# AgoraIO-Community/Solo

Hardware: AMD Instinct MI355X
Metric: 40 ms frames/sec (encode+decode) per GPU; concurrent real-time WB streams @1/2/4/8 MI355X (higher is better)
Workload: dtype int32 fixed point (int16 PCM, Q-format arithmetic, bit-exact); 1 GPU; BASELINE configs[2]: 4096 synthetic 16 kHz WB streams, full encode -> two-description bitstream -...; streams_per_gpu=4096, input_workers=16, launch=single process

## Files before the change

solo_amd/csrc/solo_enc_nsq_row.h:

```cpp
#pragma once
#include <stddef.h>
#include "solo_enc_state.h"

#define SX_JOINT_LAMBDA 90000
#define SX_DD_MASK (SX_DD_DELAY - 1)

#if SX_NLANES == 1
#define RW_NL 12
#define RW_NS 12
#define RW_FORK(l) for (int l = 0; l < 12; l++)
#define RW_LI(l) (l)
#define RW_SI(l) (l)
#define RW_ONCE(l) 1
#define RW_IS_C(l) 1
#define RW_IS_S(l) 1
#else
#define RW_NL 1
#define RW_NS 1
#define RW_FORK(l) for (int l = SX_LANE, once_ = 1; once_; once_ = 0)
#define RW_LI(l) 0
#define RW_SI(l) 0
#define RW_ONCE(l) 1
#define RW_IS_C(l) 1
#define RW_IS_S(l) 1
#endif
#define RW_T(l) ((l) >> 2)
#define RW_K(l) ((l) & 3)
#define RW_TT(l) (RW_T(l) > 2 ? 0 : RW_T(l))
#define RW_LIVE(l) (RW_T(l) < 3)
#define RW_UNI(arr) ((arr)[0])

#if SX_NLANES == 1
#define RWK_GATHER(dst, src, idx) { i32 o_[12]; for (int q_ = 0; q_ < 12; q_++) o_[q_] = (src)[q_]; for (int q_ = 0; q_ < 12; q_++) (dst)[q_] = o_[(q_ & ~3) | (idx)[q_]]; }
#define RWK_ARG_(val, mv, mi, CMP) { for (int b_ = 0; b_ < 12; b_ += 4) { i32 bv_ = (val)[b_]; int bi_ = 0;                         \
        for (int q_ = 1; q_ < 4; q_++) if ((val)[b_ + q_] CMP bv_) { bv_ = (val)[b_ + q_]; bi_ = q_; }                                \
        for (int q_ = 0; q_ < 4; q_++) { (mv)[b_ + q_] = bv_; (mi)[b_ + q_] = bi_; } } }
#define RWK_ARGMIN(val, mv, mi) RWK_ARG_(val, mv, mi, <)
#define RWK_ARGMAX(val, mv, mi) RWK_ARG_(val, mv, mi, >)
#define RWK_SUM(val, out) { for (int b_ = 0; b_ < 12; b_ += 4) { const i32 s_ = sx_add(sx_add((val)[b_], (val)[b_ + 1]), sx_add((val)[b_ + 2], (val)[b_ + 3])); \
        for (int q_ = 0; q_ < 4; q_++) (out)[b_ + q_] = s_; } }
#define RWK_PERM(LV, idx) { i32 o_[12]; for (int q_ = 0; q_ < 12; q_++) o_[q_] = LV(q_); for (int q_ = 0; q_ < 12; q_++) LV(q_) = o_[(q_ & ~3) | (idx)[q_]]; }
#define RWK_PICK(dst, src, idx) RWK_GATHER(dst, src, idx)
#define RWS_PICK(dst, src, idx) RWK_GATHER(dst, src, idx)
#define RWS_ARGMIN(val, mv, mi) RWK_ARGMIN(val, mv, mi)
#define RWS_ARGMAX(val, mv, mi) RWK_ARGMAX(val, mv, mi)
#define RWS_SUM(val, out) RWK_SUM(val, out)
#define RWS_PERM(LV, idx) RWK_PERM(LV, idx)
#define RWT_FROM(dst, src, T) { i32 o_[4]; for (int q_ = 0; q_ < 4; q_++) o_[q_] = (src)[4 * (T) + q_]; for (int q_ = 0; q_ < 12; q_++) (dst)[q_] = o_[q_ & 3]; }
#define RWT_TO0(dst, src, T) { for (int q_ = 0; q_ < 4; q_++) (dst)[q_] = (src)[4 * (T) + q_]; }
#define RWT_SUM(dst, src) { i32 o_[4]; for (int q_ = 0; q_ < 4; q_++) o_[q_] = sx_add(sx_add((src)[q_], (src)[4 + q_]), (src)[8 + q_]); for (int q_ = 0; q_ < 12; q_++) (dst)[q_] = o_[q_ & 3]; }
#define RWT_OR(dst, src) { i32 o_[4]; for (int q_ = 0; q_ < 4; q_++) o_[q_] = (src)[q_] | (src)[4 + q_] | (src)[8 + q_]; for (int q_ = 0; q_ < 12; q_++) (dst)[q_] = o_[q_ & 3]; }
#else
#define RW_DPP(v, ctrl) __builtin_amdgcn_update_dpp(0, (v), (ctrl), 0xf, 0xf, true)
#define RW_SHR(n) (0x110 + (n))
#define RW_SHL(n) (0x100 + (n))
#define RW_ROR(n) (0x120 + (n))
SX_HD i32 rwk_sel(i32 v, i32 idx) {
    const i32 b0 = RW_DPP(v, 0x00), b1 = RW_DPP(v, 0x55), b2 = RW_DPP(v, 0xAA), b3 = RW_DPP(v, 0xFF);
    const bool o_ = (idx & 1) != 0, h_ = (idx & 2) != 0;
    const i32 lo_ = o_ ? b1 : b0, hi_ = o_ ? b3 : b2;
    return h_ ? hi_ : lo_;
}
SX_HD i32 rwk_from(i32 v, i32 src) { return __builtin_amdgcn_ds_bpermute((int)((((threadIdx.x & ~3u) | (u32)src)) << 2), v); }
SX_HD i32 rwk_first_(bool eq) {
    const unsigned long long b_ = __builtin_amdgcn_ballot_w64(eq);
    return (i32)__builtin_ctz((u32)(b_ >> (threadIdx.x & 60u)) & 15u);
}
SX_HD i32 rwk_min_(i32 v) { v = sx_min(v, RW_DPP(v, 0xB1)); return sx_min(v, RW_DPP(v, 0x4E)); }
SX_HD i32 rwk_max_(i32 v) { v = sx_max(v, RW_DPP(v, 0xB1)); return sx_max(v, RW_DPP(v, 0x4E)); }
SX_HD i32 rwk_or_(i32 v) { v |= RW_DPP(v, 0xB1); return v | RW_DPP(v, 0x4E); }
SX_HD i32 rwk_sum_(i32 v) { v = sx_add(v, RW_DPP(v, 0xB1)); return sx_add(v, RW_DPP(v, 0x4E)); }
SX_HD i32 rwk_pick_(i32 v, i32 idx) { return rwk_or_((i32)(threadIdx.x & 3u) == idx ? v : 0); }
#define RWS_ARGMIN(val, mv, mi) { const i32 m_ = rwk_min_((val)[0]); (mv)[0] = m_; (mi)[0] = rwk_first_((val)[0] == m_); }
#define RWS_ARGMAX(val, mv, mi) { const i32 m_ = rwk_max_((val)[0]); (mv)[0] = m_; (mi)[0] = rwk_first_((val)[0] == m_); }
#define RWS_PICK(dst, src, idx) { (dst)[0] = rwk_pick_((src)[0], (idx)[0]); }
#define RWS_SUM(val, out) { (out)[0] = rwk_sum_((val)[0]); }
#define RWS_PERM(LV, idx) { LV(0) = rwk_from(LV(0), (idx)[0]); }
#if defined(__HIP_DEVICE_COMPILE__) && !defined(RW_CENTRE_SERIAL)
#define RW_ROW_C 1
#endif
#define RWK_GATHER(dst, src, idx) { (dst)[0] = rwk_sel((src)[0], (idx)[0]); }
#define RWK_PICK(dst, src, idx) RWS_PICK(dst, src, idx)
#define RWK_PERM(LV, idx) RWS_PERM(LV, idx)
#define RWK_ARGMIN(val, mv, mi) RWS_ARGMIN(val, mv, mi)
#define RWK_ARGMAX(val, mv, mi) RWS_ARGMAX(val, mv, mi)
SX_HD i32 rwt_from0(i32 v) { const u32 t_ = threadIdx.x & 12u; const i32 a_ = RW_DPP(v, RW_SHR(4)), b_ = RW_DPP(v, RW_SHR(8)); return t_ == 4u ? a_ : (t_ == 8u ? b_ : v); }
SX_HD i32 rwt_from1(i32 v) { const u32 t_ = threadIdx.x & 12u; const i32 a_ = RW_DPP(v, RW_SHL(4)), b_ = RW_DPP(v, RW_SHR(4)); return t_ == 0u ? a_ : (t_ == 8u ? b_ : v); }
SX_HD i32 rwt_from2(i32 v) { const u32 t_ = threadIdx.x & 12u; const i32 a_ = RW_DPP(v, RW_SHL(8)), b_ = RW_DPP(v, RW_SHL(4)); return t_ == 0u ? a_ : (t_ == 4u ? b_ : v); }
#define RWT_FROM(dst, src, T) { (dst)[0] = (T) == 0 ? rwt_from0((src)[0]) : ((T) == 1 ? rwt_from1((src)[0]) : rwt_from2((src)[0])); }
#define RWT_TO0(dst, src, T) { (dst)[0] = __builtin_amdgcn_mov_dpp((src)[0], RW_SHL(4 * (T)), 0xf, 0x1, false); }
#define RWT_SUM(dst, src) { const i32 v_ = (threadIdx.x & 12u) == 12u ? 0 : (src)[0]; \
        (dst)[0] = sx_add(sx_add(v_, RW_DPP(v_, RW_ROR(4))), sx_add(RW_DPP(v_, RW_ROR(8)), RW_DPP(v_, RW_ROR(12)))); }
#define RWT_OR(dst, src) { const i32 v_ = (threadIdx.x & 12u) == 12u ? 0 : (src)[0]; \
        (dst)[0] = (v_ | RW_DPP(v_, RW_ROR(4))) | (RW_DPP(v_, RW_ROR(8)) | RW_DPP(v_, RW_ROR(12))); }
#endif
#ifndef RW_ROW_C
#define RW_ROW_C 0
#endif

struct alignas(16) SxRowCell { i32 w0, w1, w2, w3; };
struct alignas(16) SxRowV4 { i32 x, y, z, w; };
SX_HD i32 rw_cell_x(const SxRowCell& c) { return (i32)((u32)sx_shl(c.w1 >> 26, 16) | ((u32)c.w0 >> 16)); }
SX_HD i32 rw_cell_xq(const SxRowCell& c) { return (i32)(i16)c.w0; }
SX_HD i32 rw_cell_pred_Q16(const SxRowCell& c) { return sx_shl(c.w1, 6); }

static_assert(sizeof(((SxNsqOut*)0)->q[0]) >= SX_FRAME + 3 && offsetof(SxNsqOut, q) % 4 == 0 && sizeof(((SxNsqOut*)0)->q[0]) % 4 == 0,
              "a side track's pulses are emitted with 4-byte stores: three bytes of padding behind every row");
#define SX_TAPL_N (SX_SUBFR + SX_LTP_ORDER - 1)
#define SX_TAPS_N (SX_SUBFR + 2)
#define RW_CA 0
#define RW_CAR (SX_LPC)
#define RW_CB (RW_CAR + SX_SHAPE_ORDER)
#define RW_CM (RW_CB + SX_LTP_ORDER)
#define RW_NCOEF ((RW_CM + 9 + 3) & ~3)
struct alignas(16) SxRowWorkBody {
    struct { i32 tapL[SX_TAPL_N + 1];
             i32 tapS[SX_TAPS_N + 1]; } win[SX_N_TRACKS];
    i32 xsc[SX_SUBFR];
    alignas(16) i32 coef[RW_NCOEF];
    alignas(16) i32 mdc[8];
    i32 gfac[SX_N_TRACKS][2 * SX_NB_SUBFR];
    i32 lagk[SX_NB_SUBFR];
#if SX_NLANES == 1
    SxRowCell ring_emu[SX_DD_DELAY * 12];
#endif
};
constexpr bool rw_stride_ok(int stride, int row) {
    bool used[64] = {};
    for (int s = 0; s < 4; s++)
        for (int t = 0; t < 3; t++) {
            const int b = (s * stride + t * row) % 64;
            if (used[b]) return false;
            used[b] = true;
        }
    return true;
}
constexpr int rw_work_pad_words(int body_words) {
    int pad = 0;
    while ((body_words + pad) % 4 != 0 || !rw_stride_ok(body_words + pad, SX_TAPL_N + SX_TAPS_N + 2)) pad++;
    return pad;
}
#if SX_NLANES == 1
struct alignas(16) SxRowWork : SxRowWorkBody {};
#else
struct alignas(16) SxRowWork : SxRowWorkBody { i32 pad_[rw_work_pad_words((int)(sizeof(SxRowWorkBody) / 4))]; };
static_assert(rw_stride_ok((int)(sizeof(SxRowWork) / 4), SX_TAPL_N + SX_TAPS_N + 2) && sizeof(SxRowWork) % 16 == 0, "LDS stride of the per-stream records");
#endif

SX_HD i32 sx_mul_lambda(i32 x) { return sx_add(x, sx_smulw_pre(x, (i32)((u32)(SX_JOINT_LAMBDA - 65536) << 16))); }
static_assert(SX_JOINT_LAMBDA - 65536 > 0 && SX_JOINT_LAMBDA - 65536 < 32768, "lambda split");

SX_HD void sx_nsq_rdcx1(i32 r_Q10, i32 r_p_Q10, i32 inv_of_delta_Q16, i32 Lambda_Q10, i32 offset_Q10, i32* cRdInd, i32* cQ10) {
    r_p_Q10 = sx_smulww(inv_of_delta_Q16, r_p_Q10);
    r_Q10 = sx_sub(r_Q10, offset_Q10);
    r_p_Q10 = sx_sub(r_p_Q10, offset_Q10);
    r_Q10 = sx_limit(r_Q10, -(64 << 10), 64 << 10);
    const bool lo = r_Q10 < -1536, hi = r_Q10 > 512;
    const i32 rq = sx_shl(sx_rshift_round(r_Q10, 10), 10);
    const i32 q1 = (lo | hi) ? rq : -1024;
    const i32 q2 = lo ? sx_add(rq, 1024) : (hi ? sx_sub(rq, 1024) : 0);
    const i32 e1 = sx_sub(r_p_Q10, q1), e2 = sx_sub(r_p_Q10, q2);
    const i32 a1 = sx_add(q1, offset_Q10), a2 = sx_add(q2, offset_Q10);
    const i32 rd1 = sx_smlabb(sx_mul(hi ? a1 : sx_neg(a1), Lambda_Q10), e1, e1) >> 10;
    const i32 rd2 = sx_smlabb(sx_mul(lo ? sx_neg(a2) : a2, Lambda_Q10), e2, e2) >> 10;
    const bool first = rd1 < rd2;
    cQ10[0] = first ? a1 : a2;
    cQ10[1] = first ? a2 : a1;
    cRdInd[0] = first ? rd1 : rd2;
    cRdInd[1] = first ? rd2 : rd1;
}

SX_HD i32 sx_nsq_center_rd1(i32 q_Q10, i32 r_temp_Q10, i32 offset_Q10, i32 Lambda_Q10) {
    const i32 e = sx_sub(r_temp_Q10, q_Q10);
    const i32 a = sx_add(q_Q10, offset_Q10);
    return sx_smlabb(sx_mul(q_Q10 < 0 ? sx_neg(a) : a, Lambda_Q10), e, e) >> 10;
}

#if defined(__HIP_DEVICE_COMPILE__) && defined(RW_MARKS)
#define RW_MARK(name) { __builtin_amdgcn_sched_barrier(0); asm volatile("; RW_MARK " name); __builtin_amdgcn_sched_barrier(0); }
#else
#define RW_MARK(name)
#endif
#if defined(__HIP_DEVICE_COMPILE__)
#define SX_OPAQUE(x) asm volatile("" : "+v"(x))
#define SX_SCHED_FENCE() __builtin_amdgcn_sched_barrier(0)
#define SX_LAMBDA_INLINE __attribute__((always_inline))
#else
#define SX_OPAQUE(x)
#define SX_SCHED_FENCE()
#define SX_LAMBDA_INLINE
#endif

#if defined(__HIP_DEVICE_COMPILE__) && defined(SX_GROUP)
#define SX_NSQ_FN __device__ __forceinline__
#else
#define SX_NSQ_FN SX_FN
#endif
typedef i32 __attribute__((aligned(1))) rw_i32u;
SX_HD int rw_phys(int L, int base) { const int p_ = L + base; return p_ >= 4 * SX_FRAME ? p_ - 4 * SX_FRAME : (p_ >= 2 * SX_FRAME ? p_ - 2 * SX_FRAME : p_); }

#define SX_AT(T, ubase, off) (*(T*)((char*)(ubase) + (size_t)(u32)(off)))
SX_NSQ_FN void sx_nsq_del_dec(char* Pu, u32 pOff, const SxNsqIn* c, char* Ou, u32 oOff, SxRowWork* w, SxRowCell* ringu, u32 rlane, int rstride) {
    SX_IN_LDS(w);
    SxNsqPersist* P = (SxNsqPersist*)(Pu + pOff);
    SxNsqOut* out = (SxNsqOut*)(Ou + oOff);
    const int voiced = c->sigtype == 0;
    const i32 offset_Q10 = T_quant_offsets_Q10[c->sigtype * 2 + c->QuantOffsetType];
    int lagC = P->trk[0].s.lagPrev;
    const int hbase = P->trk[0].s.histBase;
    const int cur0 = SX_FRAME - hbase;
    int smpl_buf_idx = 0;
    int decisionDelay = sx_min(SX_DD_DELAY, SX_SUBFR);
    if (voiced) {
        for (int k = 0; k < SX_NB_SUBFR; k++) decisionDelay = sx_min(decisionDelay, c->pitchL[k] - SX_LTP_ORDER / 2 - 1);
    } else if (lagC > 0) {
        decisionDelay = sx_min(decisionDelay, lagC - SX_LTP_ORDER / 2 - 1);
    }
    const int LSF_interpolation_flag = c->NLSFInterpCoef_Q2 == 4 ? 0 : 1;
#define RW_CELL(pos_, lane_) SX_AT(SxRowCell, ringu, ((u32)((pos_) * rstride) + rlane + (u32)(lane_)) * (u32)sizeof(SxRowCell))
#if defined(__HIP_DEVICE_COMPILE__) && !defined(SX_RING_TEMPORAL)
    typedef int rw_v4i_ __attribute__((ext_vector_type(4)));
#define RW_CELL_LD(dst_, pos_, lane_) { const rw_v4i_ v_ = __builtin_nontemporal_load((const rw_v4i_*)&RW_CELL(pos_, lane_)); \
        (dst_).w0 = v_.x; (dst_).w1 = v_.y; (dst_).w2 = v_.z; (dst_).w3 = v_.w; }
#define RW_CELL_ST(pos_, lane_, src_) { rw_v4i_ v_; v_.x = (src_).w0; v_.y = (src_).w1; v_.z = (src_).w2; v_.w = (src_).w3; \
        __builtin_nontemporal_store(v_, (rw_v4i_*)&RW_CELL(pos_, lane_)); }
#else
#define RW_CELL_LD(dst_, pos_, lane_) (dst_) = RW_CELL(pos_, lane_);
#define RW_CELL_ST(pos_, lane_, src_) RW_CELL(pos_, lane_) = (src_);
#endif

    i32 sAR2[RW_NL][SX_SHAPE_ORDER], sLPC[RW_NL][SX_LPC];
    i32 LF_AR[RW_NL], Seed[RW_NL], RD[RW_NL], lastShp[RW_NL];
    i32 Seed2[RW_NS], SeedInit2[RW_NS], linLo[RW_NS], linHi[RW_NS];
    i32 lagT[RW_NL], prevInv[RW_NL], gadj[RW_NL];
    u32 pTrk[RW_NL], oX[RW_NL];
    i32 LTP_pred[RW_NL], LPC_pred[RW_NL], n_AR[RW_NL], n_LF[RW_NL], rD[RW_NL], rC[RW_NS], dith[RW_NS];
    i32 cInc[RW_NL][2], cQ10[RW_NL][2];
    i32 p1q0[RW_NS], p1q1[RW_NS], p1r0[RW_NS], p1r1[RW_NS], p2q0[RW_NS], p2q1[RW_NS], p2r0[RW_NS], p2r1[RW_NS];
    SxRowCell qA[RW_NL], qB[RW_NL];
    i32 jv[RW_NS], mv[RW_NS], mi[RW_NS], mv2[RW_NS], mi2[RW_NS], tS[RW_NS], tS2[RW_NS], par[RW_NS], csrc[RW_NS], csel[RW_NS], c0[RW_NS], c1[RW_NS], nrep[RW_NS], gq[RW_NS];
    i32 tT[RW_NL], tT2[RW_NL], myRand[RW_NL];
#pragma unroll
    for (int a = 0; a < RW_NS; a++) {
        Seed2[a] = SeedInit2[a] = linLo[a] = linHi[a] = dith[a] = rC[a] = 0;
        jv[a] = mv[a] = mi[a] = mv2[a] = mi2[a] = tS[a] = tS2[a] = par[a] = csrc[a] = csel[a] = c0[a] = c1[a] = nrep[a] = gq[a] = 0;
        p1q0[a] = p1q1[a] = p1r0[a] = p1r1[a] = p2q0[a] = p2q1[a] = p2r0[a] = p2r1[a] = 0;
    }
#pragma unroll
    for (int a = 0; a < RW_NL; a++) {
        lagT[a] = prevInv[a] = tT[a] = tT2[a] = myRand[a] = 0;
        gadj[a] = 65536;
        pTrk[a] = oX[a] = 0u;
#pragma unroll
        for (int j = 0; j < SX_SHAPE_ORDER; j++) sAR2[a][j] = 0;
#pragma unroll
        for (int j = 0; j < SX_LPC; j++) sLPC[a][j] = 0;
        LF_AR[a] = Seed[a] = RD[a] = lastShp[a] = LTP_pred[a] = LPC_pred[a] = n_AR[a] = n_LF[a] = rD[a] = 0;
#pragma unroll
        for (int j = 0; j < 2; j++) cInc[a][j] = cQ10[a][j] = 0;
        qA[a].w0 = qA[a].w1 = qA[a].w2 = qA[a].w3 = 0;
        qB[a] = qA[a];
    }

    {
        SX_PAR(i, SX_N_TRACKS * SX_NB_SUBFR) {
            const int t = i / SX_NB_SUBFR, kq = i - t * SX_NB_SUBFR;
            w->gfac[t][kq] = P->trk[t].s.gadjPrev[kq];
            w->gfac[t][SX_NB_SUBFR + kq] = 65536;
        }
        SX_PAR(i, SX_NB_SUBFR) w->lagk[i] = c->pitchL[i];
        const i32 inv_gain_p1_Q16 = sx_inverse32_varQ(sx_max(c->DeltaGains_Q16, 1), 32);
        const i32 inv_gain_p2_Q16 = 65536 - inv_gain_p1_Q16;
        const i32 DeltaGains_p1_Q16 = sx_inverse32_varQ(sx_max(inv_gain_p1_Q16, 1), 32);
        const i32 DeltaGains_p2_Q16 = sx_inverse32_varQ(sx_max(inv_gain_p2_Q16, 1), 32);
        const i32 inv_of_delta_p1_Q16 = sx_inverse32_varQ(sx_max(DeltaGains_p1_Q16, 1), 32);
        const i32 inv_of_delta_p2_Q16 = sx_inverse32_varQ(sx_max(DeltaGains_p2_Q16, 1), 32);
        const i32 offset_p1_Q10 = sx_smulww(inv_gain_p1_Q16, offset_Q10);
        const i32 offset_p2_Q10 = sx_smulww(inv_gain_p2_Q16, offset_Q10);
        RW_FORK(l) {
            if (l == 0) {
                w->mdc[0] = inv_gain_p1_Q16; w->mdc[1] = inv_of_delta_p1_Q16; w->mdc[2] = offset_p1_Q10; w->mdc[3] = DeltaGains_p1_Q16;
                w->mdc[4] = inv_gain_p2_Q16; w->mdc[5] = inv_of_delta_p2_Q16; w->mdc[6] = offset_p2_Q10; w->mdc[7] = DeltaGains_p2_Q16;
                w->coef[RW_CM + 6] = c->Lambda_Q10;
                w->coef[RW_CM + 7] = offset_p1_Q10 + offset_p2_Q10;
            }
        }
        RW_FORK(l) {
            const int li = RW_LI(l), si = RW_SI(l), tt = RW_TT(l), k = RW_K(l), t = RW_T(l);
            pTrk[li] = pOff + (u32)(offsetof(SxNsqPersist, trk) + (size_t)tt * sizeof(SxNsqTrack));
            oX[li] = t == 0 ? oOff + (u32)offsetof(SxNsqOut, r) - (u32)(4 * cur0) : oOff + (u32)(offsetof(SxNsqOut, q) + (size_t)(tt - 1) * (SX_FRAME + 4)) - (u32)cur0;
            const SxNSQ* n = &SX_AT(SxNSQ, Pu, pTrk[li] + (u32)offsetof(SxNsqTrack, s));
            lagT[li] = n->lagPrev;
            prevInv[li] = n->prev_inv_gain_Q16;
            Seed2[si] = SeedInit2[si] = (k + c->Seed) & 3;
            linLo[si] = linHi[si] = k * 0x55555555;
            Seed[li] = (k + c->Seed) & 3;
            RD[li] = 0;
            LF_AR[li] = n->sLF_AR_shp_Q12;
            lastShp[li] = SX_AT(i32, Pu, pTrk[li] + (u32)(offsetof(SxNsqTrack, shp) + (size_t)rw_phys(SX_FRAME - 1, hbase) * 4));
#pragma unroll
            for (int i = 0; i < SX_LPC; i++) sLPC[li][i] = n->sLPC_Q14[SX_MAX_LPC - 1 - i];
#pragma unroll
            for (int i = 0; i < SX_SHAPE_ORDER; i++) sAR2[li][i] = n->sAR2_Q14[i];
        }
        wv_sync();
    }
    RW_FORK(l) {
        const int l0 = (SX_DD_MASK + decisionDelay) & SX_DD_MASK;
        qA[RW_LI(l)] = RW_CELL(l0, l);
    }
    int sLTP_shp_buf_idx = SX_FRAME, sLTP_buf_idx = SX_FRAME;
    int subfr = 0;
    int rewhite_k = 0;

#define RW_LIN_SLOT(lo_, hi_, pos_) ((int)((((pos_) < 16 ? (u32)(lo_) : (u32)(hi_)) >> (2 * ((pos_) & 15))) & 3u))
#define RW_EMIT_OUT(l_, li_, cell_, e4_, WIDE)                                                                               \
    {                                                                                                                        \
        if (WIDE) SX_AT(rw_i32u, Ou, oX[li_] + (RW_T(l_) == 0 ? (u32)(e4_) : (u32)(e4_) >> 2)) = rw_cell_x(cell_);           \
        else if (RW_T(l_) == 0) SX_AT(i32, Ou, oX[li_] + (u32)(e4_)) = rw_cell_x(cell_);                                     \
        else SX_AT(i8, Ou, oX[li_] + ((u32)(e4_) >> 2)) = (i8)rw_cell_x(cell_);                                              \
        SX_AT(i16, Pu + offsetof(SxNsqTrack, xq), pTrk[li_] + ((u32)(e4_) >> 1)) = (i16)rw_cell_xq(cell_);                    \
        SX_AT(i32, Pu + offsetof(SxNsqTrack, shp), pTrk[li_] + (u32)(e4_)) = (cell_).w2;                                      \
    }
#define RW_FLUSH(wlo_, whi_, pos0_)                                                                                          \
    RW_FORK(l) {                                                                                                             \
        const int li = RW_LI(l);                                                                                             \
        if (RW_LIVE(l)) {                                                                                                    \
            for (int base = RW_K(l); base < decisionDelay; base += 16) {                                                     \
                SxRowCell cl[4];                                                                                             \
                _Pragma("unroll") for (int u = 0; u < 4; u++) {                                                              \
                    const int i = base + 4 * u;                                                                              \
                    const int rp = (smpl_buf_idx + decisionDelay - 1 - i) & SX_DD_MASK;                                      \
                    if (i < decisionDelay) cl[u] = RW_CELL(rp, (l & ~3) | RW_LIN_SLOT(wlo_, whi_, rp));                      \
                }                                                                                                            \
                _Pragma("unroll") for (int u = 0; u < 4; u++) {                                                              \
                    const int i = base + 4 * u;                                                                              \
                    if (i < decisionDelay) RW_EMIT_OUT(l, li, cl[u], 4 * (cur0 + (pos0_) + i), false)                                  \
                }                                                                                                            \
            }                                                                                                                \
        }                                                                                                                    \
    }

    for (int k = 0; k < SX_NB_SUBFR; k++) {
        const i16* A_Q12 = c->PredCoef_Q12[(k >> 1) | (1 - LSF_interpolation_flag)];
        const i16* B_Q14 = &c->LTPCoef_Q14[k * SX_LTP_ORDER];
        const i16* AR_shp_Q13 = &c->AR2_Q13[k * SX_SHAPE_ORDER];
        i32 HarmShapeFIRPacked_Q14 = c->HarmShapeGain_Q14[k] >> 2;
        HarmShapeFIRPacked_Q14 |= sx_shl(c->HarmShapeGain_Q14[k] >> 1, 16);
        const i32 Tilt_Q14 = c->Tilt_Q14[k], LF_shp_Q14 = c->LF_shp_Q14[k], Gain_Q16 = c->Gains_Q16[k];
        int rewhite = 0;
        i32 inv_gain_Q16 = sx_inverse32_varQ(sx_max(Gain_Q16, 1), 32);
        inv_gain_Q16 = sx_min(inv_gain_Q16, 32767);
        i32 inv_gain_Q32 = sx_shl(inv_gain_Q16, 16);
        if (k == 0) inv_gain_Q32 = sx_shl(sx_smulwb(inv_gain_Q32, c->LTP_scale_Q14), 2);
        if (voiced) {
            lagC = c->pitchL[k];
            RW_FORK(l) { lagT[RW_LI(l)] = lagC; }
            if ((k & (3 - sx_shl(LSF_interpolation_flag, 1))) == 0) {
                if (k == 2) {
                    subfr = 0;
                    RWT_FROM(jv, RD, 0)
                    RWS_ARGMIN(jv, mv, mi)
                    RW_FORK(l) {
                        if (RW_K(l) != mi[RW_SI(l)]) RD[RW_LI(l)] += SX_I32_MAX >> 4;
                    }
                    RWS_PICK(tS, linLo, mi)
                    RWS_PICK(tS2, linHi, mi)
                    wv_sync();
                    RW_FLUSH(tS[RW_SI(l)], tS2[RW_SI(l)], k * SX_SUBFR - decisionDelay)
                    wv_sync();
                }
                const int lag = lagC;
                const int start_idx = SX_FRAME - lag - SX_LPC - SX_LTP_ORDER / 2;
                const int len = SX_FRAME - start_idx;
                const int per = (len + SX_NLANES - 1) / SX_NLANES;
                const int n0 = SX_LANE * per, n1 = sx_min(len, n0 + per);
                i32 Ac[SX_LPC];
// ... 143 lines not shown
#else
#define RW_CF_STAGE(j0_, j1_) SX_SCHED_FENCE(); RW_CF_LOAD(j0_, j1_) SX_SCHED_FENCE();
#endif
            const i32 *Apre = cf + RW_CA, *ARpre = cf + RW_CAR, *Bpre = cf + RW_CB;
            constexpr int G1 = (RW_CAR + 3) / 4, G2 = (RW_CB + 3) / 4;
            i32 curL[RW_NL][SX_LTP_ORDER], curS[RW_NL][3], tmp1[RW_NL], tmp2[RW_NL], nAR_[RW_NL];
            const i32 x_sc_Q10 = w->xsc[i];
            RW_FORK(l) {
                const int li = RW_LI(l), si = RW_SI(l), tt = RW_TT(l);
#pragma unroll
                for (int j = 0; j < SX_LTP_ORDER; j++) curL[li][j] = w->win[tt].tapL[i + (SX_LTP_ORDER - 1) - j];
#pragma unroll
                for (int j = 0; j < 3; j++) curS[li][j] = w->win[tt].tapS[i + 2 - j];
                if (RW_ONCE(l)) {
                    Seed2[si] = sx_rand(Seed2[si]);
                    dith[si] = Seed2[si] >> 31;
                }
                const SxRowV4 v_ = *(const SxRowV4*)__builtin_assume_aligned((const char*)w->mdc + co_ + 4 * sd[li], 16);
                my_inv_gain[li] = v_.x; my_inv_of_delta[li] = v_.y; my_offset[li] = v_.z; my_DG[li] = v_.w;
                LPC_pred[li] = 0;
            }
            RW_CF_STAGE(0, G1)
            RW_CF_STAGE(G1, G2)
#pragma unroll
            for (int j = 0; j < SX_LPC; j++) {
                RW_FORK(l) { const int li = RW_LI(l); LPC_pred[li] = sx_smlaw_pre(LPC_pred[li], sLPC[li][j], Apre[j]); }
            }
            RW_CF_STAGE(G2, RW_NCOEF / 4)
            const i32 warp_pre = cf[RW_CM + 0], Tilt_pre = cf[RW_CM + 1], LFb_pre = cf[RW_CM + 2], LFt_pre = cf[RW_CM + 3], Hb_pre = cf[RW_CM + 4], Ht_pre = cf[RW_CM + 5];
#define RW_STEP(body_) { RW_FORK(l) { const int li = RW_LI(l); body_ } }
            i32 dd_[RW_NL], mm_[RW_NL];
            RW_STEP(dd_[li] = sx_smulw_pre(sAR2[li][0], warp_pre);)
            RW_STEP(tmp2[li] = sx_add(sLPC[li][0], dd_[li]);)
            RW_STEP(dd_[li] = sx_sub(sAR2[li][1], tmp2[li]); mm_[li] = sx_smulw_pre(tmp2[li], ARpre[0]);)
            RW_STEP(dd_[li] = sx_smulw_pre(dd_[li], warp_pre); nAR_[li] = mm_[li];)
            RW_STEP(tmp1[li] = sx_add(sAR2[li][0], dd_[li]); sAR2[li][0] = tmp2[li];)
#pragma unroll
            for (int j = 2; j < SX_SHAPE_ORDER; j += 2) {
                RW_STEP(dd_[li] = sx_sub(sAR2[li][j], tmp1[li]); mm_[li] = sx_smulw_pre(tmp1[li], ARpre[j - 1]);)
                RW_STEP(dd_[li] = sx_smulw_pre(dd_[li], warp_pre); nAR_[li] = sx_add(nAR_[li], mm_[li]);)
                RW_STEP(tmp2[li] = sx_add(sAR2[li][j - 1], dd_[li]); sAR2[li][j - 1] = tmp1[li];)
                RW_STEP(dd_[li] = sx_sub(sAR2[li][j + 1], tmp2[li]); mm_[li] = sx_smulw_pre(tmp2[li], ARpre[j]);)
                RW_STEP(dd_[li] = sx_smulw_pre(dd_[li], warp_pre); nAR_[li] = sx_add(nAR_[li], mm_[li]);)
                RW_STEP(tmp1[li] = sx_add(sAR2[li][j], dd_[li]); sAR2[li][j] = tmp2[li];)
            }
            RW_FORK(l) {
                const int li = RW_LI(l), si = RW_SI(l);
                const i32 dither = dith[si];
                sAR2[li][SX_SHAPE_ORDER - 1] = tmp1[li];
                i32 n_AR_Q10 = sx_smlaw_pre(nAR_[li], tmp1[li], ARpre[SX_SHAPE_ORDER - 1]);
                n_AR_Q10 = n_AR_Q10 >> 1;
                n_AR_Q10 = sx_smlaw_pre(n_AR_Q10, LF_AR[li], Tilt_pre);
                i32 n_LF_Q10 = sx_shl(sx_smulw_pre(lastShp[li], LFb_pre), 2);
                n_LF_Q10 = sx_smlaw_pre(n_LF_Q10, LF_AR[li], LFt_pre);
                n_AR[li] = n_AR_Q10;
                n_LF[li] = n_LF_Q10;
                i32 LTP_pred_Q14 = 0;
#pragma unroll
                for (int j = 0; j < SX_LTP_ORDER; j++) LTP_pred_Q14 = sx_smlaw_pre(LTP_pred_Q14, curL[li][j], Bpre[j]);
                i32 n_LTP_Q14 = sx_smulw_pre(sx_add(curS[li][0], curS[li][2]), Hb_pre);
                n_LTP_Q14 = sx_smlaw_pre(n_LTP_Q14, curS[li][1], Ht_pre);
                n_LTP_Q14 = sx_shl(n_LTP_Q14, 6);
                i32 tmp = sx_sub(LTP_pred_Q14, n_LTP_Q14) >> 4;
                tmp = sx_add(tmp, LPC_pred[li]);
                tmp = sx_sub(tmp, n_AR_Q10);
                tmp = sx_sub(tmp, n_LF_Q10);
                i32 r_Q10 = sx_sub(x_sc_Q10, tmp);
                Seed[li] = sx_rand(Seed[li]);
                r_Q10 = (r_Q10 ^ dither) - dither;
                LTP_pred[li] = LTP_pred_Q14;
                rD[li] = r_Q10;
            }
            RW_MARK("B")
            const i32 Lambda_Q10 = cf[RW_CM + 6], offsum = cf[RW_CM + 7], Gain_s = cf[RW_CM + 8];
            RWT_FROM(rC, rD, 0)
            RW_FORK(l) {
                const int li = RW_LI(l), si = RW_SI(l);
                if (RW_IS_S(l)) {
                    const i32 r_md_Q10 = sx_smulww(my_inv_gain[li], rC[si]);
                    sx_nsq_rdcx1(r_md_Q10, rD[li], my_inv_of_delta[li], Lambda_Q10, my_offset[li], cInc[li], cQ10[li]);
                }
            }
            RW_MARK("C")
            i32 wpk[RW_NS], ccInc[RW_NS][2], ccQ10[RW_NS][2];
#if RW_ROW_C
            {
                const u32 t4_ = threadIdx.x & 12u;
                const i32 q0_ = cQ10[0][0], q1_ = cQ10[0][1], r0_ = cInc[0][0], r1_ = cInc[0][1];
                i32 x1q = q1_, x1r = r1_, x2q = q1_, x2r = r1_;
                x1q = __builtin_amdgcn_update_dpp(x1q, q0_, RW_SHL(4), 0xf, 0x1, false);  x1r = __builtin_amdgcn_update_dpp(x1r, r0_, RW_SHL(4), 0xf, 0x1, false);
                x2q = __builtin_amdgcn_update_dpp(x2q, q0_, RW_SHL(8), 0xf, 0x1, false);  x2r = __builtin_amdgcn_update_dpp(x2r, r0_, RW_SHL(8), 0xf, 0x1, false);
                x1q = __builtin_amdgcn_update_dpp(x1q, q0_, RW_SHR(4), 0xf, 0x4, false);  x1r = __builtin_amdgcn_update_dpp(x1r, r0_, RW_SHR(4), 0xf, 0x4, false);
                x2q = __builtin_amdgcn_update_dpp(x2q, q1_, RW_SHL(4), 0xf, 0x2, false);  x2r = __builtin_amdgcn_update_dpp(x2r, r1_, RW_SHL(4), 0xf, 0x2, false);
                x1q = __builtin_amdgcn_update_dpp(x1q, q1_, RW_SHR(8), 0xf, 0x8, false);  x1r = __builtin_amdgcn_update_dpp(x1r, r1_, RW_SHR(8), 0xf, 0x8, false);
                x2q = __builtin_amdgcn_update_dpp(x2q, q0_, RW_SHR(4), 0xf, 0x8, false);  x2r = __builtin_amdgcn_update_dpp(x2r, r0_, RW_SHR(4), 0xf, 0x8, false);
                const i32 rc3_ = RW_DPP(rD[0], RW_SHR(12));
                const i32 r_temp = sx_sub(t4_ == 12u ? rc3_ : rC[0], offsum);
                const i32 qx = sx_add(x1q, x2q);
                const i32 rd_ = sx_add(sx_add(sx_nsq_center_rd1(qx, r_temp, offsum, Lambda_Q10), sx_mul_lambda(x1r)), sx_mul_lambda(x2r));
                const i32 k0_ = (i32)(((u32)rd_ << 2) | (t4_ >> 2));
                const i32 ka_ = RW_DPP(k0_, RW_ROR(4)), kb_ = RW_DPP(k0_, RW_ROR(8)), kc_ = RW_DPP(k0_, RW_ROR(12));
                const i32 lo1 = sx_min(k0_, ka_), hi1 = sx_max(k0_, ka_), lo2 = sx_min(kb_, kc_), hi2 = sx_max(kb_, kc_);
                const i32 m1 = sx_min(lo1, lo2), m2 = sx_min(sx_max(lo1, lo2), sx_min(hi1, hi2));
                const u32 w1 = (u32)m1 & 3u, w2 = (u32)m2 & 3u;
                tS[0] = (i32)(w1 | (w2 << 2));
                ccInc[0][0] = m1 >> 2;
                ccInc[0][1] = m2 >> 2;
#ifdef RW_CQ_SELECT
                const i32 p1q1_ = RW_DPP(q1_, RW_SHL(4)), p2q1_ = RW_DPP(q1_, RW_SHL(8));
                ccQ10[0][0] = sx_add(((0xAu >> w1) & 1u) ? p1q1_ : x1q, ((0x6u >> w1) & 1u) ? p2q1_ : x2q);
                ccQ10[0][1] = sx_add(((0xAu >> w2) & 1u) ? p1q1_ : x1q, ((0x6u >> w2) & 1u) ? p2q1_ : x2q);
#else
                const u32 lb_ = (threadIdx.x & 0x33u) << 2;
                ccQ10[0][0] = __builtin_amdgcn_ds_bpermute((int)((w1 << 4) | lb_), qx);
                ccQ10[0][1] = __builtin_amdgcn_ds_bpermute((int)((w2 << 4) | lb_), qx);
#endif
                (void)wpk;
            }
#else
            { i32 a_[RW_NL], b_[RW_NL], c_[RW_NL], d_[RW_NL];
#pragma unroll
              for (int q_ = 0; q_ < RW_NL; q_++) { a_[q_] = cQ10[q_][0]; b_[q_] = cQ10[q_][1]; c_[q_] = cInc[q_][0]; d_[q_] = cInc[q_][1]; }
              RWT_TO0(p1q0, a_, 1) RWT_TO0(p1q1, b_, 1) RWT_TO0(p1r0, c_, 1) RWT_TO0(p1r1, d_, 1)
              RWT_TO0(p2q0, a_, 2) RWT_TO0(p2q1, b_, 2) RWT_TO0(p2r0, c_, 2) RWT_TO0(p2r1, d_, 2) }
            RW_FORK(l) {
              if (RW_IS_C(l)) {
                const int li = RW_LI(l), si = RW_SI(l);
                const i32 off = offsum;
                const i32 qx0 = p1q0[si] + p2q0[si], qx1 = p1q1[si] + p2q1[si], qx2 = p1q0[si] + p2q1[si], qx3 = p1q1[si] + p2q0[si];
                const i32 r_temp = sx_sub(rD[li], off);
                const i32 l1r0 = sx_mul_lambda(p1r0[si]), l1r1 = sx_mul_lambda(p1r1[si]), l2r0 = sx_mul_lambda(p2r0[si]), l2r1 = sx_mul_lambda(p2r1[si]);
                i32 rdx0 = sx_nsq_center_rd1(qx0, r_temp, off, Lambda_Q10), rdx1 = sx_nsq_center_rd1(qx1, r_temp, off, Lambda_Q10);
                i32 rdx2 = sx_nsq_center_rd1(qx2, r_temp, off, Lambda_Q10), rdx3 = sx_nsq_center_rd1(qx3, r_temp, off, Lambda_Q10);
                rdx0 = sx_add(sx_add(rdx0, l1r0), l2r0);
                rdx1 = sx_add(sx_add(rdx1, l1r1), l2r1);
                rdx2 = sx_add(sx_add(rdx2, l1r0), l2r1);
                rdx3 = sx_add(sx_add(rdx3, l1r1), l2r0);
                const i32 m1 = sx_min(sx_min(rdx0, rdx1), sx_min(rdx2, rdx3));
                const bool e0 = rdx0 == m1, e1 = rdx1 == m1, e2 = rdx2 == m1;
                const int w1 = e0 ? 0 : (e1 ? 1 : (e2 ? 2 : 3));
                const i32 q_w1 = e0 ? qx0 : (e1 ? qx1 : (e2 ? qx2 : qx3));
                const i32 x0 = w1 == 0 ? SX_I32_MAX : rdx0, x1 = w1 == 1 ? SX_I32_MAX : rdx1, x2 = w1 == 2 ? SX_I32_MAX : rdx2, x3 = w1 == 3 ? SX_I32_MAX : rdx3;
                const i32 m2 = sx_min(sx_min(x0, x1), sx_min(x2, x3));
                const bool f0 = x0 == m2, f1 = x1 == m2, f2 = x2 == m2;
                const int w2 = f0 ? 0 : (f1 ? 1 : (f2 ? 2 : 3));
                const i32 q_w2 = f0 ? qx0 : (f1 ? qx1 : (f2 ? qx2 : qx3));
                ccInc[si][0] = m1;
                ccInc[si][1] = m2;
                ccQ10[si][0] = q_w1;
                ccQ10[si][1] = q_w2;
                wpk[si] = w1 | (w2 << 2);
              }
            }
            RWT_FROM(tS, wpk, 0)
#endif
            RW_FORK(l) {
                const int li = RW_LI(l), si = RW_SI(l), t = RW_T(l);
                const u32 mtab = t == 1 ? 0xAu : 0x6u;
                const bool ca = ((mtab >> (tS[si] & 3)) & 1u) != 0, cb = ((mtab >> ((tS[si] >> 2) & 3)) & 1u) != 0;
                const i32 a0 = cInc[li][0], a1 = cInc[li][1], d0 = cQ10[li][0], d1 = cQ10[li][1];
                const bool ctr = t == 0;
                cInc[li][0] = ctr ? ccInc[si][0] : (ca ? a1 : a0);  cInc[li][1] = ctr ? ccInc[si][1] : (cb ? a1 : a0);
                cQ10[li][0] = ctr ? ccQ10[si][0] : (ca ? d1 : d0); cQ10[li][1] = ctr ? ccQ10[si][1] : (cb ? d1 : d0);
                const i32 cand0 = sx_add(RD[li], cInc[li][0]);
                tT[li] = sx_add(cand0, sx_smulw_pre(cand0, lamT[li]));
            }
            RWT_SUM(jv, tT)
            smpl_buf_idx = smpl_new;
            RW_MARK("E")
            i32 pen[RW_NS];
            {
                const i32 PEN = SX_I32_MAX >> 4;
                RWS_ARGMIN(jv, mv, mi)
                const bool written = k * SX_SUBFR + i >= decisionDelay;
                RW_FORK(l) {
                    if (RW_ONCE(l)) gq[RW_SI(l)] = RW_LIN_SLOT(linLo[RW_SI(l)], linHi[RW_SI(l)], last_smple_idx);
                    tT[RW_LI(l)] = qc[RW_LI(l)].w3;
                }
                RWK_GATHER(tT2, tT, gq)
                RW_FORK(l) { myRand[RW_LI(l)] = written ? tT2[RW_LI(l)] : 0; }
                RWK_PICK(tT2, myRand, mi)
                RW_FORK(l) { tT[RW_LI(l)] = (myRand[RW_LI(l)] ^ tT2[RW_LI(l)]) != 0 ? 1 : 0; }
                RWT_OR(tS2, tT)
                RW_FORK(l) {
                    if (RW_IS_C(l)) {
                        const int li = RW_LI(l), si = RW_SI(l);
                        pen[si] = tS2[si] ? PEN : 0;
                        par[si] = RW_K(l); csrc[si] = RW_K(l); csel[si] = 0;
                        const i32 rp_ = sx_add(RD[li], pen[si]);
                        c0[si] = sx_add(rp_, cInc[li][0]); c1[si] = sx_add(rp_, cInc[li][1]);
                    }
                }
                RWS_SUM(tS2, nrep)
                RWS_ARGMIN(c1, mv2, mi2)
#if SX_NLANES == 1
                int RandSyncCtl = RW_UNI(nrep);
                do {
                    RWS_ARGMAX(c0, mv, mi)
                    RWS_PICK(gq, par, mi2)
                    RW_FORK(l) {
                        const int si = RW_SI(l);
                        const bool rep_ = (mv2[si] < mv[si]) & (RW_K(l) == mi[si]);
                        par[si] = rep_ ? gq[si] : par[si]; csrc[si] = rep_ ? mi2[si] : csrc[si]; csel[si] = rep_ ? 1 : csel[si]; c0[si] = rep_ ? mv2[si] : c0[si];
                    }
                } while (--RandSyncCtl > 0);
#else
                i32 RandSyncCtl = nrep[0];
                do {
                    RWS_ARGMAX(c0, mv, mi)
                    RWS_PICK(gq, par, mi2)
                    const bool rep_ = (mv2[0] < mv[0]) & ((i32)(threadIdx.x & 3u) == mi[0]);
                    par[0] = rep_ ? gq[0] : par[0]; csrc[0] = rep_ ? mi2[0] : csrc[0]; csel[0] = rep_ ? 1 : csel[0]; c0[0] = rep_ ? mv2[0] : c0[0];
                } while (--RandSyncCtl > 0);
#endif
                RW_FORK(l) { if (RW_ONCE(l)) tS[RW_SI(l)] = par[RW_SI(l)] | (csrc[RW_SI(l)] << 2) | (csel[RW_SI(l)] << 4); }
                RWT_FROM(tS2, tS, 0)
                RW_FORK(l) { if (RW_ONCE(l)) { const int si = RW_SI(l); par[si] = tS2[si] & 3; csrc[si] = (tS2[si] >> 2) & 3; csel[si] = (tS2[si] >> 4) & 1; } }
            }
            RW_MARK("M")
            i32 cand1RD[RW_NL], cand1Q10[RW_NL], penT[RW_NL];
            {
                RW_FORK(l) {
                    const int li = RW_LI(l);
                    penT[li] = RW_T(l) == 0 ? pen[RW_SI(l)] : 0;
                    cand1RD[li] = sx_add(sx_add(RD[li], penT[li]), cInc[li][1]); cand1Q10[li] = cQ10[li][1];
                }
#define RW_LV_C1RD(q_) cand1RD[q_]
#define RW_LV_C1Q10(q_) cand1Q10[q_]
#define RW_LV_LPCP(q_) LPC_pred[q_]
#define RW_LV_NAR(q_) n_AR[q_]
#define RW_LV_NLF(q_) n_LF[q_]
#define RW_LV_DITH(q_) dith[q_]
                RWK_PERM(RW_LV_C1RD, csrc) RWK_PERM(RW_LV_C1Q10, csrc)
                RWK_PERM(RW_LV_LPCP, csrc) RWK_PERM(RW_LV_NAR, csrc) RWK_PERM(RW_LV_NLF, csrc) RWS_PERM(RW_LV_DITH, csrc)
#define RW_LV_SEED2(q_) Seed2[q_]
#define RW_LV_SEEDI(q_) SeedInit2[q_]
#define RW_LV_LINLO(q_) linLo[q_]
#define RW_LV_LINHI(q_) linHi[q_]
#define RW_LV_SEED(q_) Seed[q_]
                RWS_PERM(RW_LV_SEED2, par) RWS_PERM(RW_LV_SEEDI, par) RWS_PERM(RW_LV_LINLO, par) RWS_PERM(RW_LV_LINHI, par) RWK_PERM(RW_LV_SEED, par)
#pragma unroll
                for (int j = 0; j < SX_SHAPE_ORDER; j++) {
#define RW_LV_SAR2(q_) sAR2[q_][j]
                    RWK_PERM(RW_LV_SAR2, par)
                }
#pragma unroll
                for (int j = SX_LPC - 1; j > 0; j--) {
#if SX_NLANES == 1
                    { i32 o_[12]; for (int q_ = 0; q_ < 12; q_++) o_[q_] = sLPC[q_][j - 1]; for (int q_ = 0; q_ < 12; q_++) sLPC[q_][j] = o_[(q_ & ~3) | par[q_]]; }
#else
#pragma unroll
                    for (int q_ = 0; q_ < RW_NL; q_++) sLPC[q_][j] = rwk_from(sLPC[q_][j - 1], par[0]);
#endif
                }
            }
            RW_MARK("D")
            i32 fRD[RW_NL], fQ0[RW_NL], cXq14[RW_NL], cShp[RW_NL], cExc10[RW_NL], cX[RW_NL];
            RW_FORK(l) {
                const int li = RW_LI(l), si = RW_SI(l), t = RW_T(l);
                const i32 dither = dith[si];
                const bool sel = csel[si] != 0;
                const i32 Q10 = sel ? cand1Q10[li] : cQ10[li][0];
                fRD[li] = sel ? cand1RD[li] : sx_add(sx_add(RD[li], penT[li]), cInc[li][0]);
                i32 Q = (Q10 ^ dither) - dither;
                const bool ctr = t == 0;
                fQ0[li] = ctr ? Q10 >> 10 : (i32)(i8)(sx_sub(Q10, my_offset[li]) >> 10);
                cX[li] = ctr ? Q : fQ0[li];
                Q = ctr ? Q : sx_smulww(my_DG[li], Q);
                const i32 LPC_exc_Q10 = Q + sx_rshift_round(LTP_pred[li], 4);
                const i32 xq_Q10 = sx_add(LPC_exc_Q10, LPC_pred[li]);
                const i32 sLF_AR_shp_Q10 = sx_sub(xq_Q10, n_AR[li]);
                cShp[li] = sx_sub(sLF_AR_shp_Q10, n_LF[li]);
                LF_AR[li] = sx_shl(sLF_AR_shp_Q10, 2);
                cXq14[li] = sx_shl(xq_Q10, 4);
                cExc10[li] = LPC_exc_Q10;
                tT[li] = sx_add(fRD[li], sx_smulw_pre(fRD[li], lamT[li]));
            }
            RWT_SUM(jv, tT)
            RW_MARK("F")
            RWS_ARGMIN(jv, mv, mi)
            {
                RW_FORK(l) { if (RW_ONCE(l)) tS[RW_SI(l)] = RW_LIN_SLOT(linLo[RW_SI(l)], linHi[RW_SI(l)], last_smple_idx); }
                RWS_PICK(gq, tS, mi)
                const bool crossed = subfr > 0 && i < decisionDelay;
                RW_FORK(l) {
                    const int li = RW_LI(l);
                    if (emitted && RW_K(l) == gq[RW_SI(l)] && RW_LIVE(l)) {
                        const u32 e4 = (u32)(4 * (cur0 + k * SX_SUBFR + i - decisionDelay));
                        const i32 p16 = rw_cell_pred_Q16(qc[li]);
                        const i32 gx = crossed ? gadj[li] : 65536;
                        RW_EMIT_OUT(l, li, qc[li], e4, true)
                        SX_AT(i32, Pu + offsetof(SxNsqTrack, sLTP_Q16), pTrk[li] + e4 + (u32)dL4) = p16;
                        const u32 iL = (u32)(i + wb[li]), iS = iL - 1u;
                        w->win[RW_T(l)].tapL[iL < (u32)SX_TAPL_N ? iL : (u32)SX_TAPL_N] = sx_smulww(gx, p16);
                        w->win[RW_T(l)].tapS[iS < (u32)SX_TAPS_N ? iS : (u32)SX_TAPS_N] = sx_smulww(gx, qc[li].w2);
                    }
                }
            }
            RW_MARK("G")
            RW_FORK(l) {
                const int li = RW_LI(l), si = RW_SI(l), kk = RW_K(l);
                sLPC[li][0] = cXq14[li];
                lastShp[li] = cShp[li];
                Seed[li] = sx_add(Seed[li], fQ0[li]);
                RD[li] = fRD[li];
                SxRowCell cell;
                const i32 xq16 = sx_sat16(sx_rshift_round(sx_smulww(cXq14[li] >> 4, Gain_s), 10));
                cell.w0 = (i32)(((u32)xq16 & 0xFFFFu) | ((u32)cX[li] << 16));
                cell.w1 = (i32)(((u32)cExc10[li] & 0x03FFFFFFu) | (((u32)cX[li] << 10) & 0xFC000000u));
                cell.w2 = cShp[li];
                cell.w3 = Seed[li];
                if (RW_LIVE(l)) RW_CELL_ST(smpl_buf_idx, l, cell)
                if (RW_ONCE(l)) {
                    const u32 m = 3u << (2 * (smpl_buf_idx & 15));
                    if (smpl_buf_idx < 16) linLo[si] = (i32)(((u32)linLo[si] & ~m) | (((u32)kk * 0x55555555u) & m));
                    else linHi[si] = (i32)(((u32)linHi[si] & ~m) | (((u32)kk * 0x55555555u) & m));
                }
            }
            RW_MARK("Z")
            wv_sync_lds();
        };
        static_assert(SX_SUBFR % 2 == 0, "two samples per iteration");
        for (int i = 0; i < SX_SUBFR; i += 2) {
            sample_step(i, qA, qB);
            sample_step(i + 1, qB, qA);
        }
        sLTP_shp_buf_idx += SX_SUBFR;
        sLTP_buf_idx += SX_SUBFR;
        subfr++;
    }

    RWT_FROM(jv, RD, 0)
    RWS_ARGMIN(jv, mv, mi)
    RWS_PICK(tS, SeedInit2, mi)
    RW_FORK(l) { if (l == 0) out->Seed = tS[RW_SI(l)]; }
    RWS_PICK(tS, linLo, mi)
    RWS_PICK(tS2, linHi, mi)
    wv_sync();
    RW_FLUSH(tS[RW_SI(l)], tS2[RW_SI(l)], SX_FRAME - decisionDelay)
    wv_sync();
    RW_FORK(l) {
        const int li = RW_LI(l);
        if (RW_K(l) == mi[RW_SI(l)] && RW_LIVE(l)) {
            SxNSQ* n = &SX_AT(SxNSQ, Pu, pTrk[li] + (u32)offsetof(SxNsqTrack, s));
#pragma unroll
            for (int i = 0; i < SX_MAX_LPC; i++) n->sLPC_Q14[i] = (SX_MAX_LPC - 1 - i) < SX_LPC ? sLPC[li][SX_MAX_LPC - 1 - i] : 0;
#pragma unroll
            for (int i = 0; i < SX_SHAPE_ORDER; i++) n->sAR2_Q14[i] = sAR2[li][i];
            n->sLF_AR_shp_Q12 = LF_AR[li];
            n->lagPrev = c->pitchL[SX_NB_SUBFR - 1];
            n->prev_inv_gain_Q16 = prevInv[li];
            n->histBase = cur0;
#pragma unroll
            for (int kq = 0; kq < SX_NB_SUBFR; kq++) n->gadjPrev[kq] = w->gfac[RW_T(l)][SX_NB_SUBFR + kq];
        }
    }
    wv_sync();
#undef RW_EMIT_OUT
#undef RW_FLUSH
#undef RW_CELL
#undef RW_CELL_LD
#undef RW_CELL_ST
#undef SX_AT
}
```

Before: 3.927 million 40ms packets/s (encode+decode).

## Pack NSQ survivor plan into one word and recover seed via LCG inverse

```diff
diff --git a/solo_amd/csrc/solo_enc_nsq_row.h b/solo_amd/csrc/solo_enc_nsq_row.h
--- a/solo_amd/csrc/solo_enc_nsq_row.h
+++ b/solo_amd/csrc/solo_enc_nsq_row.h
@@ -41,6 +41,7 @@
         for (int q_ = 0; q_ < 4; q_++) (out)[b_ + q_] = s_; } }
 #define RWK_PERM(LV, idx) { i32 o_[12]; for (int q_ = 0; q_ < 12; q_++) o_[q_] = LV(q_); for (int q_ = 0; q_ < 12; q_++) LV(q_) = o_[(q_ & ~3) | (idx)[q_]]; }
 #define RWK_PICK(dst, src, idx) RWK_GATHER(dst, src, idx)
+#define RWK_GATHER_X(dst, src, idx) RWK_GATHER(dst, src, idx)
 #define RWS_PICK(dst, src, idx) RWK_GATHER(dst, src, idx)
 #define RWS_ARGMIN(val, mv, mi) RWK_ARGMIN(val, mv, mi)
 #define RWS_ARGMAX(val, mv, mi) RWK_ARGMAX(val, mv, mi)
@@ -80,6 +81,7 @@
 #define RW_ROW_C 1
 #endif
 #define RWK_GATHER(dst, src, idx) { (dst)[0] = rwk_sel((src)[0], (idx)[0]); }
+#define RWK_GATHER_X(dst, src, idx) { (dst)[0] = rwk_from((src)[0], (idx)[0]); }
 #define RWK_PICK(dst, src, idx) RWS_PICK(dst, src, idx)
 #define RWK_PERM(LV, idx) RWS_PERM(LV, idx)
 #define RWK_ARGMIN(val, mv, mi) RWS_ARGMIN(val, mv, mi)
@@ -176,6 +178,8 @@
     return sx_smlabb(sx_mul(q_Q10 < 0 ? sx_neg(a) : a, Lambda_Q10), e, e) >> 10;
 }
 
+constexpr u32 rw_inv_u32(u32 a) { u32 x = a; for (int i = 0; i < 5; i++) x *= 2u - a * x; return x; }
+
 #if defined(__HIP_DEVICE_COMPILE__) && defined(RW_MARKS)
 #define RW_MARK(name) { __builtin_amdgcn_sched_barrier(0); asm volatile("; RW_MARK " name); __builtin_amdgcn_sched_barrier(0); }
 #else
@@ -231,19 +235,19 @@
 
     i32 sAR2[RW_NL][SX_SHAPE_ORDER], sLPC[RW_NL][SX_LPC];
     i32 LF_AR[RW_NL], Seed[RW_NL], RD[RW_NL], lastShp[RW_NL];
-    i32 Seed2[RW_NS], SeedInit2[RW_NS], linLo[RW_NS], linHi[RW_NS];
+    i32 Seed2[RW_NS], linLo[RW_NS], linHi[RW_NS];
     i32 lagT[RW_NL], prevInv[RW_NL], gadj[RW_NL];
     u32 pTrk[RW_NL], oX[RW_NL];
     i32 LTP_pred[RW_NL], LPC_pred[RW_NL], n_AR[RW_NL], n_LF[RW_NL], rD[RW_NL], rC[RW_NS], dith[RW_NS];
     i32 cInc[RW_NL][2], cQ10[RW_NL][2];
     i32 p1q0[RW_NS], p1q1[RW_NS], p1r0[RW_NS], p1r1[RW_NS], p2q0[RW_NS], p2q1[RW_NS], p2r0[RW_NS], p2r1[RW_NS];
     SxRowCell qA[RW_NL], qB[RW_NL];
-    i32 jv[RW_NS], mv[RW_NS], mi[RW_NS], mv2[RW_NS], mi2[RW_NS], tS[RW_NS], tS2[RW_NS], par[RW_NS], csrc[RW_NS], csel[RW_NS], c0[RW_NS], c1[RW_NS], nrep[RW_NS], gq[RW_NS];
+    i32 jv[RW_NS], mv[RW_NS], mi[RW_NS], mv2[RW_NS], mi2[RW_NS], tS[RW_NS], tS2[RW_NS], par[RW_NS], csrc[RW_NS], csel[RW_NS], plan[RW_NS], c0[RW_NS], c1[RW_NS], nrep[RW_NS], gq[RW_NS];
     i32 tT[RW_NL], tT2[RW_NL], myRand[RW_NL];
 #pragma unroll
     for (int a = 0; a < RW_NS; a++) {
-        Seed2[a] = SeedInit2[a] = linLo[a] = linHi[a] = dith[a] = rC[a] = 0;
-        jv[a] = mv[a] = mi[a] = mv2[a] = mi2[a] = tS[a] = tS2[a] = par[a] = csrc[a] = csel[a] = c0[a] = c1[a] = nrep[a] = gq[a] = 0;
+        Seed2[a] = linLo[a] = linHi[a] = dith[a] = rC[a] = 0;
+        jv[a] = mv[a] = mi[a] = mv2[a] = mi2[a] = tS[a] = tS2[a] = par[a] = csrc[a] = csel[a] = plan[a] = c0[a] = c1[a] = nrep[a] = gq[a] = 0;
         p1q0[a] = p1q1[a] = p1r0[a] = p1r1[a] = p2q0[a] = p2q1[a] = p2r0[a] = p2r1[a] = 0;
     }
 #pragma unroll
@@ -292,7 +296,7 @@
             const SxNSQ* n = &SX_AT(SxNSQ, Pu, pTrk[li] + (u32)offsetof(SxNsqTrack, s));
             lagT[li] = n->lagPrev;
             prevInv[li] = n->prev_inv_gain_Q16;
-            Seed2[si] = SeedInit2[si] = (k + c->Seed) & 3;
+            Seed2[si] = (k + c->Seed) & 3;
             linLo[si] = linHi[si] = k * 0x55555555;
             Seed[li] = (k + c->Seed) & 3;
             RD[li] = 0;
@@ -602,6 +606,11 @@
                 }
             }
             RW_MARK("C")
+            RW_FORK(l) {
+                if (RW_ONCE(l)) gq[RW_SI(l)] = RW_LIN_SLOT(linLo[RW_SI(l)], linHi[RW_SI(l)], last_smple_idx);
+                tT[RW_LI(l)] = qc[RW_LI(l)].w3;
+            }
+            RWK_GATHER_X(myRand, tT, gq)
             i32 wpk[RW_NS], ccInc[RW_NS][2], ccQ10[RW_NS][2];
 #if RW_ROW_C
             {
@@ -688,27 +697,22 @@
             RWT_SUM(jv, tT)
             smpl_buf_idx = smpl_new;
             RW_MARK("E")
-            i32 pen[RW_NS];
+            i32 penT[RW_NL], c0i[RW_NS];
             {
                 const i32 PEN = SX_I32_MAX >> 4;
                 RWS_ARGMIN(jv, mv, mi)
                 const bool written = k * SX_SUBFR + i >= decisionDelay;
-                RW_FORK(l) {
-                    if (RW_ONCE(l)) gq[RW_SI(l)] = RW_LIN_SLOT(linLo[RW_SI(l)], linHi[RW_SI(l)], last_smple_idx);
-                    tT[RW_LI(l)] = qc[RW_LI(l)].w3;
-                }
-                RWK_GATHER(tT2, tT, gq)
-                RW_FORK(l) { myRand[RW_LI(l)] = written ? tT2[RW_LI(l)] : 0; }
+                RW_FORK(l) { myRand[RW_LI(l)] = written ? myRand[RW_LI(l)] : 0; }
                 RWK_PICK(tT2, myRand, mi)
                 RW_FORK(l) { tT[RW_LI(l)] = (myRand[RW_LI(l)] ^ tT2[RW_LI(l)]) != 0 ? 1 : 0; }
                 RWT_OR(tS2, tT)
                 RW_FORK(l) {
                     if (RW_IS_C(l)) {
                         const int li = RW_LI(l), si = RW_SI(l);
-                        pen[si] = tS2[si] ? PEN : 0;
-                        par[si] = RW_K(l); csrc[si] = RW_K(l); csel[si] = 0;
-                        const i32 rp_ = sx_add(RD[li], pen[si]);
-                        c0[si] = sx_add(rp_, cInc[li][0]); c1[si] = sx_add(rp_, cInc[li][1]);
+                        penT[li] = (RW_T(l) == 0 && tS2[si] != 0) ? PEN : 0;
+                        plan[si] = RW_K(l) * 5;
+                        const i32 rp_ = sx_add(RD[li], penT[li]);
+                        c0[si] = c0i[si] = sx_add(rp_, cInc[li][0]); c1[si] = sx_add(rp_, cInc[li][1]);
                     }
                 }
                 RWS_SUM(tS2, nrep)
@@ -717,35 +721,34 @@
                 int RandSyncCtl = RW_UNI(nrep);
                 do {
                     RWS_ARGMAX(c0, mv, mi)
-                    RWS_PICK(gq, par, mi2)
+                    RWS_PICK(gq, plan, mi2)
                     RW_FORK(l) {
                         const int si = RW_SI(l);
                         const bool rep_ = (mv2[si] < mv[si]) & (RW_K(l) == mi[si]);
-                        par[si] = rep_ ? gq[si] : par[si]; csrc[si] = rep_ ? mi2[si] : csrc[si]; csel[si] = rep_ ? 1 : csel[si]; c0[si] = rep_ ? mv2[si] : c0[si];
+                        plan[si] = rep_ ? ((gq[si] & 3) | (mi2[si] << 2) | 16) : plan[si]; c0[si] = rep_ ? mv2[si] : c0[si];
                     }
                 } while (--RandSyncCtl > 0);
 #else
                 i32 RandSyncCtl = nrep[0];
+                const i32 take1_ = (mi2[0] << 2) | 16;
                 do {
                     RWS_ARGMAX(c0, mv, mi)
-                    RWS_PICK(gq, par, mi2)
+                    RWS_PICK(gq, plan, mi2)
                     const bool rep_ = (mv2[0] < mv[0]) & ((i32)(threadIdx.x & 3u) == mi[0]);
-                    par[0] = rep_ ? gq[0] : par[0]; csrc[0] = rep_ ? mi2[0] : csrc[0]; csel[0] = rep_ ? 1 : csel[0]; c0[0] = rep_ ? mv2[0] : c0[0];
+                    plan[0] = rep_ ? ((gq[0] & 3) | take1_) : plan[0]; c0[0] = rep_ ? mv2[0] : c0[0];
                 } while (--RandSyncCtl > 0);
 #endif
-                RW_FORK(l) { if (RW_ONCE(l)) tS[RW_SI(l)] = par[RW_SI(l)] | (csrc[RW_SI(l)] << 2) | (csel[RW_SI(l)] << 4); }
-                RWT_FROM(tS2, tS, 0)
+                RWT_FROM(tS2, plan, 0)
                 RW_FORK(l) { if (RW_ONCE(l)) { const int si = RW_SI(l); par[si] = tS2[si] & 3; csrc[si] = (tS2[si] >> 2) & 3; csel[si] = (tS2[si] >> 4) & 1; } }
             }
             RW_MARK("M")
-            i32 cand1RD[RW_NL], cand1Q10[RW_NL], penT[RW_NL];
+            i32 cand1Q10[RW_NL];
             {
                 RW_FORK(l) {
                     const int li = RW_LI(l);
-                    penT[li] = RW_T(l) == 0 ? pen[RW_SI(l)] : 0;
-                    cand1RD[li] = sx_add(sx_add(RD[li], penT[li]), cInc[li][1]); cand1Q10[li] = cQ10[li][1];
-                }
-#define RW_LV_C1RD(q_) cand1RD[q_]
+                    cand1Q10[li] = cQ10[li][1];
+                }
+#define RW_LV_C1RD(q_) c1[q_]
 #define RW_LV_C1Q10(q_) cand1Q10[q_]
 #define RW_LV_LPCP(q_) LPC_pred[q_]
 #define RW_LV_NAR(q_) n_AR[q_]
@@ -754,11 +757,10 @@
                 RWK_PERM(RW_LV_C1RD, csrc) RWK_PERM(RW_LV_C1Q10, csrc)
                 RWK_PERM(RW_LV_LPCP, csrc) RWK_PERM(RW_LV_NAR, csrc) RWK_PERM(RW_LV_NLF, csrc) RWS_PERM(RW_LV_DITH, csrc)
 #define RW_LV_SEED2(q_) Seed2[q_]
-#define RW_LV_SEEDI(q_) SeedInit2[q_]
 #define RW_LV_LINLO(q_) linLo[q_]
 #define RW_LV_LINHI(q_) linHi[q_]
 #define RW_LV_SEED(q_) Seed[q_]
-                RWS_PERM(RW_LV_SEED2, par) RWS_PERM(RW_LV_SEEDI, par) RWS_PERM(RW_LV_LINLO, par) RWS_PERM(RW_LV_LINHI, par) RWK_PERM(RW_LV_SEED, par)
+                RWS_PERM(RW_LV_SEED2, par) RWS_PERM(RW_LV_LINLO, par) RWS_PERM(RW_LV_LINHI, par) RWK_PERM(RW_LV_SEED, par)
 #pragma unroll
                 for (int j = 0; j < SX_SHAPE_ORDER; j++) {
 #define RW_LV_SAR2(q_) sAR2[q_][j]
@@ -781,7 +783,7 @@
                 const i32 dither = dith[si];
                 const bool sel = csel[si] != 0;
                 const i32 Q10 = sel ? cand1Q10[li] : cQ10[li][0];
-                fRD[li] = sel ? cand1RD[li] : sx_add(sx_add(RD[li], penT[li]), cInc[li][0]);
+                fRD[li] = sel ? c1[si] : c0i[si];
                 i32 Q = (Q10 ^ dither) - dither;
                 const bool ctr = t == 0;
                 fQ0[li] = ctr ? Q10 >> 10 : (i32)(i8)(sx_sub(Q10, my_offset[li]) >> 10);
@@ -852,7 +854,13 @@
 
     RWT_FROM(jv, RD, 0)
     RWS_ARGMIN(jv, mv, mi)
-    RWS_PICK(tS, SeedInit2, mi)
+    {
+        constexpr SxLcgMap fm_ = sx_lcg_map((u32)SX_FRAME);
+        constexpr u32 Ainv_ = rw_inv_u32(fm_.A);
+        static_assert((u32)(fm_.A * Ainv_) == 1u, "inverse of the frame's LCG multiplier");
+        RW_FORK(l) { if (RW_ONCE(l)) tS2[RW_SI(l)] = (i32)(((u32)Seed2[RW_SI(l)] - fm_.C) * Ainv_); }
+    }
+    RWS_PICK(tS, tS2, mi)
     RW_FORK(l) { if (l == 0) out->Seed = tS[RW_SI(l)]; }
     RWS_PICK(tS, linLo, mi)
     RWS_PICK(tS2, linHi, mi)
```

Result: no change. 3.961 million 40ms packets/s (encode+decode) (median of 6 runs) (+0.9%).
